# apache/bifromq

Measured on AMD Instinct MI355X. Metric: publish-topic matches/sec (whole node), higher is better.
Workload: dtype u32

## Files before the change

### bifromq_amd/csrc/bmq_dist_kernels.h

```cpp
#pragma once
#ifndef BMQ_WAVE_EMU
#include <hip/hip_runtime.h>
#endif

#include <type_traits>

#include "bmq_layout.h"
#include "bmq_batch_args.h"

namespace bmq {

#ifndef BMQ_WAVE_EMU
__device__ __forceinline__ void wave_sync() {
    __builtin_amdgcn_fence(__ATOMIC_RELEASE, "wavefront");
    __builtin_amdgcn_wave_barrier();
    __builtin_amdgcn_fence(__ATOMIC_ACQUIRE, "wavefront");
}
__device__ __forceinline__ uint32_t rank_below(unsigned long long mask) {
    return __builtin_amdgcn_mbcnt_hi((uint32_t)(mask >> 32), __builtin_amdgcn_mbcnt_lo((uint32_t)mask, 0u));
}
#endif
__device__ __forceinline__ uint32_t wave_excl_scan(uint32_t v, uint32_t lane, uint32_t& total) {
    uint32_t inc = v;
#pragma unroll
// ... 2 lines not shown
        if (lane >= (uint32_t)d) inc += o;
    }
    total = __shfl(inc, 63);
    return inc - v;
}
__device__ __forceinline__ unsigned long long wave_sum_u64(unsigned long long v) {
#pragma unroll
    for (int d = 32; d >= 1; d >>= 1) v += __shfl_xor(v, d);
    return v;
}

__device__ __forceinline__ TrieSlot unpack_slot(const uint4& a, const uint4& b) {
    TrieSlot s;
    s.parent = a.x; s.token = a.y; s.own_begin = a.z; s.own_count = a.w;
    s.hash_begin = b.x; s.hash_count = b.y; s.node = b.z; s.lit_bloom = b.w;
    return s;
}
struct Line64 {
    uint4 a0, a1, b0, b1;
};
static_assert(DICT_GROUP == 2, "a dictionary group is one Line64");
#ifndef BMQ_WAVE_EMU
__device__ __forceinline__ void load_line64(const void* p, Line64& r) {
    asm volatile("global_load_dwordx4 %0, %4, off\n\t"
                 "global_load_dwordx4 %1, %4, off offset:16\n\t"
                 "global_load_dwordx4 %2, %4, off offset:32\n\t"
                 "global_load_dwordx4 %3, %4, off offset:48\n\t"
                 "s_waitcnt vmcnt(0)"
                 : "=&v"(r.a0), "=&v"(r.a1), "=&v"(r.b0), "=&v"(r.b1)
                 : "v"(p));
}
__device__ __forceinline__ void load_line64_s(const void* sbase, uint32_t voff, Line64& r) {
    asm volatile("global_load_dwordx4 %0, %4, %5\n\t"
                 "global_load_dwordx4 %1, %4, %5 offset:16\n\t"
                 "global_load_dwordx4 %2, %4, %5 offset:32\n\t"
                 "global_load_dwordx4 %3, %4, %5 offset:48\n\t"
                 "s_waitcnt vmcnt(0)"
                 : "=&v"(r.a0), "=&v"(r.a1), "=&v"(r.b0), "=&v"(r.b1)
                 : "v"(voff), "s"(sbase));
}
#else
inline void load_line64(const void* p, Line64& r) { memcpy(&r, p, 64); }
inline void load_line64_s(const void* sbase, uint32_t voff, Line64& r) { memcpy(&r, reinterpret_cast<const uint8_t*>(sbase) + voff, 64); }
#endif
template <class ByteAt>
__device__ __forceinline__ uint32_t dict_lookup(const DistIndexView& ix, const LevelHash& h, uint32_t len,
                                                const uint32_t inl[4], uint32_t start, ByteAt&& byte_at) {
    const uint32_t tag = level_hash_tag(h);
    uint32_t g = level_hash_slot(h, len) & ix.dict_group_mask;
    auto tail_eq = [&](uint32_t pool_off) {
        bool eq = true;
        for (uint32_t i = 16; i < len && eq; i++) eq = ix.pool[pool_off + i] == byte_at(start + i);
        return eq;
    };
    for (uint32_t probes = 0; probes <= ix.dict_group_mask; probes++) {
        Line64 ln;
        load_line64(ix.dict + DICT_GROUP * (size_t)g, ln);
        const bool h0 = ln.a0.x == tag && ln.a0.z == len && ln.a1.x == inl[0] && ln.a1.y == inl[1] && ln.a1.z == inl[2] &&
                        ln.a1.w == inl[3];
        const bool h1 = ln.b0.x == tag && ln.b0.z == len && ln.b1.x == inl[0] && ln.b1.y == inl[1] && ln.b1.z == inl[2] &&
                        ln.b1.w == inl[3];
        if (h0 && (len <= 16 || tail_eq(ln.a0.w))) return ln.a0.y;
        if (h1 && (len <= 16 || tail_eq(ln.b0.w))) return ln.b0.y;
        if (ln.a0.x == 0 || ln.b0.x == 0) return TOK_UNKNOWN;
        g = (g + 1) & ix.dict_group_mask;
    }
    return TOK_UNKNOWN;
}

#ifndef BMQ_WAVE_EMU
__device__ __forceinline__ void load_slot32(const void* p, uint4& a, uint4& b) {
    asm volatile("global_load_dwordx4 %0, %2, off\n\t"
                 "global_load_dwordx4 %1, %2, off offset:16\n\t"
                 "s_waitcnt vmcnt(0)"
                 : "=&v"(a), "=&v"(b)
                 : "v"(p));
}
#else
inline void load_slot32(const void* p, uint4& a, uint4& b) {
    memcpy(&a, p, 16);
    memcpy(&b, reinterpret_cast<const uint8_t*>(p) + 16, 16);
}
#endif
template <class ByteAt>
__device__ __forceinline__ uint32_t dict_lookup_by_slot(const DistIndexView& ix, const LevelHash& h, uint32_t len, const uint32_t inl[4], uint32_t start,
                                                        ByteAt&& byte_at) {
    const uint32_t tag = level_hash_tag(h);
    uint32_t g = level_hash_slot(h, len) & ix.dict_group_mask;
    auto tail_eq = [&](uint32_t pool_off) {
        bool eq = true;
        for (uint32_t i = 16; i < len && eq; i++) eq = ix.pool[pool_off + i] == byte_at(start + i);
        return eq;
    };
    for (uint32_t probes = 0; probes <= ix.dict_group_mask; probes++) {
        const DictSlot* grp = ix.dict + DICT_GROUP * (size_t)g;
#pragma unroll
        for (uint32_t k = 0; k < DICT_GROUP; k++) {
            uint4 hd, in;
            load_slot32(grp + k, hd, in);
            if (hd.x == tag && hd.z == len && in.x == inl[0] && in.y == inl[1] && in.z == inl[2] && in.w == inl[3] && (len <= 16 || tail_eq(hd.w))) return hd.y;
            if (hd.x == 0) return TOK_UNKNOWN;
        }
        g = (g + 1) & ix.dict_group_mask;
    }
    return TOK_UNKNOWN;
}

template <class WordAt>
__device__ __forceinline__ void scan_level(uint32_t& pos, uint32_t end, bool split, WordAt&& word_at, LevelHash& h,
                                           uint32_t inl[4], uint32_t& len, bool& last) {
    h = level_hash_init();
    inl[0] = inl[1] = inl[2] = inl[3] = 0;
    len = 0;
    for (;;) {
        const uint32_t remaining = end - pos;
        if (remaining == 0) break;
        const uint32_t w = word_at(pos);
        uint32_t nb = 4;
        if (split) {
            const uint32_t x = w ^ 0x2F2F2F2Fu;
            const uint32_t z = (x - 0x01010101u) & ~x & 0x80808080u;
            if (z) nb = (uint32_t)(__ffs((int)z) - 1) >> 3;
        }
        nb = min(nb, remaining);
        if (nb) {
            const uint32_t wm = nb == 4 ? w : (w & ((1u << (8u * nb)) - 1u));
            level_hash_word(h, wm);
            if (len < 16) inl[len >> 2] = wm;
            len += nb;
            pos += nb;
        }
        if (nb < 4) break;
    }
    if (pos < end) {
        pos++;
        last = false;
    } else {
        last = true;
    }
}

__device__ __forceinline__ uint32_t global_word_at(const uint8_t* base, uint32_t p) {
    const uint32_t* a = reinterpret_cast<const uint32_t*>(base + (p & ~3u));
    return __builtin_amdgcn_alignbyte(a[1], a[0], p & 3u);
}

constexpr TenantSlot EMPTY_TENANT{0, 0, 0, 0, 0, 1, 0, 0, 0, 0, 0, 0, {0, 0, 0}, NONE};
__device__ __forceinline__ bool tenant_known(const TenantSlot& t) { return (t.hash_lo | t.hash_hi) != 0; }

__global__ __launch_bounds__(64) void k_reset(Counters* ctr, SubAlloc* subs, unsigned long long* super_sums, uint32_t n_super) {
    const uint32_t i = blockIdx.x * 64 + threadIdx.x;
    if (i < sizeof(Counters) / 8) reinterpret_cast<unsigned long long*>(ctr)[i] = 0ull;
    if (i < sizeof(SubAlloc) * 2 * N_SUB / 8) reinterpret_cast<unsigned long long*>(subs)[i] = 0ull;
    if (i < n_super) super_sums[(size_t)i * SUPER_STRIDE] = 0ull;
}

static_assert(sizeof(Counters) % 16 == 0 && sizeof(Counters) / 16 <= 64, "one wave copies the counters, 16 bytes per lane");
__global__ __launch_bounds__(64) void k_publish(const Counters* ctr, Counters* host) {
    const uint32_t i = threadIdx.x;
    if (i < sizeof(Counters) / 16) reinterpret_cast<uint4*>(host)[i] = reinterpret_cast<const uint4*>(ctr)[i];
}

struct TenantQuery {
    uint32_t beg = 0, len = 0;
    uint32_t raw[5] = {0, 0, 0, 0, 0};
    uint32_t w[4] = {0, 0, 0, 0};
// ... 367 lines not shown
```

### bifromq_amd/csrc/bmq_engine.hip

```cpp
#include <hip/hip_runtime.h>

#include <algorithm>
#include <array>
#include <chrono>
#include <condition_variable>
#include <cstdio>
#include <cstdlib>
#include <cstring>
#include <map>
#include <memory>
#include <mutex>
#include <string>
#include <string_view>
#include <thread>
#include <type_traits>
#include <vector>

#include "../../include/bmq.h"
#include "bmq_codec.h"
#include "bmq_dist_index.h"
#include "bmq_dist_kernels.h"
#include "bmq_poll_kernel.h"
#include "bmq_exec_dev.h"
#include "bmq_exec_host.h"
// ... 508 lines not shown
    S.pair_cap = S.pair_cap * 2;
    if (S.pair_cap >= 0xFFFFFFFFull) return set_err(e, BMQ_E_RANGE, "matched-range buffer exceeds 2^32 entries");
    HIPCHK(e, S.b_pairs.ensure(sizeof(MatchRange) * S.pair_cap));
    return BMQ_OK;
}
int grow_sort_list(bmq_engine* e, bmq_engine::BatchSlot& S, uint32_t sort_count) {
    S.sort_cap = std::max<uint32_t>(S.sort_cap * 2, sort_count);
    HIPCHK(e, S.b_sort_list.ensure(sizeof(uint32_t) * S.sort_cap));
    return BMQ_OK;
}

static void print_wave_debug(bmq_engine* e, bmq_engine::BatchSlot& S) {
    const BatchArgs& a = S.last;
    if (!a.dbg_wave || !a.n_blocks) return;
    std::vector<uint4> h(2 * (size_t)a.n_blocks);
    if (hipMemcpy(h.data(), a.dbg_wave, sizeof(uint4) * 2 * a.n_blocks, hipMemcpyDeviceToHost) != hipSuccess) return;
    if (a.debug_flags & 24u) {
        std::vector<std::pair<unsigned long long, int>> ev;
        unsigned long long t0 = ~0ull, t1 = 0, busy = 0;
        std::map<uint32_t, std::vector<std::pair<unsigned long long, int>>> per_simd;
        for (uint32_t i = 0; i < a.n_blocks; i++) {
            const unsigned long long st = ((unsigned long long)h[i].y << 32) | h[i].x, en = st + h[i].z;
            t0 = std::min(t0, st), t1 = std::max(t1, en), busy += h[i].z;
            ev.push_back({st, 1}), ev.push_back({en, -1});
            const uint32_t simd_key = (h[i].w >> 4) & 0xFFFFFu & ~0xCu;
            per_simd[simd_key].push_back({st, 1}), per_simd[simd_key].push_back({en, -1});
        }
        if (const char* fn = bmq_env("BMQ_CENSUS_FILE")) {
            if (FILE* f = fopen(fn, "wb")) {
                fwrite(h.data(), sizeof(uint4), a.n_blocks, f);
                fclose(f);
            }
        }
        std::sort(ev.begin(), ev.end());
        int cur = 0, peak = 0;
        for (auto& x : ev) cur += x.second, peak = std::max(peak, cur);
        int simd_peak = 0;
        double simd_peak_sum = 0;
        for (auto& kv : per_simd) {
            std::sort(kv.second.begin(), kv.second.end());
            int c = 0, pk = 0;
            for (auto& x : kv.second) c += x.second, pk = std::max(pk, c);
            simd_peak = std::max(simd_peak, pk), simd_peak_sum += pk;
        }
        fprintf(stderr, "[bmq] k_walk census: %u waves, span %llu ticks, mean wave %.0f ticks, mean resident %.0f (peak %d) waves; %zu distinct SIMD keys, peak waves on one SIMD %d (mean of peaks %.1f)\n",
                a.n_blocks, t1 - t0, (double)busy / a.n_blocks, (double)busy / (double)(t1 - t0), peak, per_simd.size(), simd_peak,
                simd_peak_sum / std::max<size_t>(per_simd.size(), 1));
        return;
    }
    if (a.debug_flags & 4u) {
        if (!BMQ_EXP_CLOCKS) {
            fprintf(stderr, "[bmq] k_expand phase clocks need a build with -DBMQ_EXP_CLOCKS=1 (tools/build_variant.sh)\n");
            return;
        }
        double p[4] = {0, 0, 0, 0};
        for (uint32_t i = 0; i < a.n_blocks; i++) p[0] += h[i].x, p[1] += h[i].y, p[2] += h[i].z, p[3] += h[i].w;
        fprintf(stderr, "[bmq] k_expand waves=%u clocks/wave: head %.0f load+order %.0f prefix %.0f generate %.0f\n", a.n_blocks,
                p[0] / a.n_blocks, p[1] / a.n_blocks, p[2] / a.n_blocks, p[3] / a.n_blocks);
        {
            std::vector<unsigned long long> tot(a.n_blocks);
            unsigned long long mx_tail = 0;
            for (uint32_t i = 0; i < a.n_blocks; i++) {
                tot[i] = (unsigned long long)h[i].x + h[i].y + h[i].z + h[i].w;
                if (i >= a.n_blocks - a.n_blocks / 10) mx_tail = std::max(mx_tail, tot[i]);
            }
            std::sort(tot.begin(), tot.end());
            fprintf(stderr, "[bmq] k_expand wave lifetimes (clocks): p50 %llu p90 %llu p99 %llu max %llu; longest among the last tenth of the blocks %llu\n",
                    tot[a.n_blocks / 2], tot[(size_t)(a.n_blocks * 0.9)], tot[(size_t)(a.n_blocks * 0.99)], tot.back(), mx_tail);
        }
        return;
    }
    double s1 = 0, s2 = 0, s3 = 0, sr = 0, si = 0;
    std::vector<uint32_t> r(a.n_blocks), c2(a.n_blocks);
    for (uint32_t i = 0; i < a.n_blocks; i++) {
        s1 += h[i].x, s2 += h[i].y, s3 += h[i].z, sr += h[i].w & 255u, si += h[i].w >> 8;
        r[i] = h[i].w & 255u, c2[i] = h[i].y;
    }
    std::sort(r.begin(), r.end());
    std::sort(c2.begin(), c2.end());
    const double n = a.n_blocks;
    {
        double pa = 0, pb = 0, pc = 0;
        for (uint32_t i = 0; i < a.n_blocks; i++) pa += h[a.n_blocks + i].x, pb += h[a.n_blocks + i].y, pc += h[a.n_blocks + i].z;
        fprintf(stderr, "[bmq] k_walk tokenise in detail: stage bytes %.0f | offsets + tenant %.0f | levels + dictionary %.0f\n", pa / n, pb / n, pc / n);
    }
    fprintf(stderr, "[bmq] k_walk waves=%u clocks/wave: tokenise %.0f walk %.0f (p50 %u p99 %u) write %.0f | rounds mean %.1f p50 %u p99 %u max %u | items/wave %.0f\n",
            a.n_blocks, s1 / n, s2 / n, c2[a.n_blocks / 2], c2[(size_t)(a.n_blocks * 0.99)], s3 / n, sr / n, r[a.n_blocks / 2],
            r[(size_t)(a.n_blocks * 0.99)], r.back(), si / n);
}

int finish_dist(bmq_engine* e, bmq_engine::BatchSlot& S, uint64_t* out_total) {
    const auto rerun = [&] {
        BatchArgs a = S.last;
        return launch_dist(e, S, a);
    };
    for (int attempt = 0; attempt < 8; attempt++) {
        HIPCHK(e, hipEventSynchronize(S.ev_done));
        if (S.last.debug_flags & 30u) print_wave_debug(e, S);
        const Counters c = *S.h_ctr;
        const uint32_t grow = c.status & (ST_RERUN | ST_NEED_SORTLIST | ST_NEED_ADJ);
        if (grow) {
            int rc;
            if ((grow & ST_NEED_PAIRS) && (rc = grow_pairs(e, S))) return rc;
            if (grow & ST_NEED_SPILL) {
                S.spill_cap = S.spill_cap * 2;
                if (S.spill_cap >= 0xFFFFFFFFull) return set_err(e, BMQ_E_RANGE, "range spill buffer exceeds 2^32 records");
                HIPCHK(e, S.b_spill.ensure(sizeof(uint4) * S.spill_cap));
            }
            if (grow & ST_NEED_SLOW) {
                S.slow_cap = std::max<uint32_t>(S.slow_cap * 2, c.slow_count);
                HIPCHK(e, S.b_slow_list.ensure(sizeof(uint32_t) * S.slow_cap));
            }
            if (grow & ST_NEED_SCRATCH) {
                S.scratch_cap = std::max<uint64_t>(S.scratch_cap * 2, c.scratch_alloc + c.scratch_alloc / 8);
                HIPCHK(e, S.b_scratch.ensure(sizeof(uint32_t) * S.scratch_cap));
            }
            if (grow & ST_NEED_ADJ) {
                S.adj_cap = (uint64_t)c.adj_bytes + c.adj_bytes / 8 + 4096;
                HIPCHK(e, S.b_c_topics.ensure(S.adj_cap + 64));
            }
            if ((grow & ST_NEED_SORTLIST) && (rc = grow_sort_list(e, S, c.sort_count))) return rc;
            if (c.sort_count) e->sort_on = true, e->sort_idle = 0;
            if (c.slow_count) e->slow_on = true, e->slow_idle = 0;
            if (c.status & ST_WANT_MIXED) e->mixed_on = true, e->mixed_idle = 0;
            if ((rc = rerun())) return rc;
            continue;
        }
        if ((c.status & ST_WANT_MIXED) && !S.ran_mixed) {
            e->mixed_on = true, e->mixed_idle = 0;
            if (int rc = rerun()) return rc;
            continue;
        }
        if (c.slow_count && !S.ran_slow) {
            e->slow_on = true, e->slow_idle = 0;
            if (int rc = rerun()) return rc;
            continue;
        }
        if (c.sort_count && !S.ran_sort && !(c.status & (ST_RANGE | ST_NOSPACE))) {
            e->sort_on = true, e->sort_idle = 0;
            HIPCHK(e, hipMemcpyAsync(S.last.ctr, S.h_ctr, sizeof(Counters), hipMemcpyHostToDevice, e->stream));
            hipLaunchKernelGGL(k_sort_rows, dim3(1024), dim3(256), 0, e->stream, S.last);
            reset_slot(e, S, e->stream);
            HIPCHK(e, hipGetLastError());
            HIPCHK(e, hipStreamSynchronize(e->stream));
        }
        if (S.ran_slow && (c.slow_count ? (e->slow_idle = 0) : ++e->slow_idle) >= REPAIR_IDLE_BATCHES) e->slow_on = false;
        if (S.ran_sort && (c.sort_count ? (e->sort_idle = 0) : ++e->sort_idle) >= REPAIR_IDLE_BATCHES) e->sort_on = false;
        if (S.ran_mixed && ++e->mixed_idle >= 8 * REPAIR_IDLE_BATCHES) e->mixed_on = false;
        S.pending = false;
        bmq_stats& st = e->stats;
        st = bmq_stats{};
        st.n_topics = S.last.n_topics;
        st.n_visit = c.n_visit;
        st.n_match = c.total_ids;
        st.n_ranges = c.n_ranges;
        st.n_slow_topics = c.slow_count;
        st.n_sorted_rows = c.sort_count;
        st.topic_bytes = c.topic_bytes;
        st.n_walked = c.n_walked ? c.n_walked : (S.last.rep ? 0u : S.last.n_topics);
        st.n_split_blocks = S.last.heavy_list ? std::min(c.heavy_count, S.last.heavy_cap) : 0u;
        if (S.last.heavy_list) {
            const double nb = S.last.n_blocks, mr = c.n_ranges / nb, mi = c.total_ids / nb;
            e->blk_mean_ranges = e->blk_mean_ranges > 0 ? 0.75 * e->blk_mean_ranges + 0.25 * mr : mr;
            e->blk_mean_ids = e->blk_mean_ids > 0 ? 0.75 * e->blk_mean_ids + 0.25 * mi : mi;
            constexpr double base = EXPAND_SPLIT_MULT_X16 / 16.0;
            if (c.heavy_count > S.last.heavy_cap) e->split_mult *= 1.25;
            else if (c.heavy_count < S.last.heavy_cap / 4) e->split_mult = std::max(base, e->split_mult / 1.05);
// ... 1359 lines not shown
```

### bifromq_amd/csrc/bmq_walk_kernel.h

```cpp
#pragma once

namespace bmq {

constexpr uint32_t WALK_MAX_TENANTS = 4;
__device__ __forceinline__ uint32_t walk_meta(uint32_t tl, uint32_t tokpos, uint32_t rem) { return tl | (tokpos << 6) | (rem << 16); }
constexpr uint32_t WALK_META_CHILD = 64u - 65536u;

#define BMQ_WALK_GEOM_DEFAULT 512, 176, 152
#define BMQ_WALK_GEOM_SMALLEST 192, 128, 128
constexpr uint32_t WALK_QC_DEFAULT = 176, WALK_PC_DEFAULT = 152, WALK_QC_SMALLEST = 128, WALK_PC_SMALLEST = 128;

template <int TC, int QC, int PC, bool MIXED> struct WalkLds {
    static constexpr uint32_t TOK = 0;
    static constexpr uint32_t STK = TOK + TC * 4;
    static constexpr uint32_t PRG = STK + QC * 8;
    static constexpr uint32_t PTP = PRG + PC * 8;
    static constexpr uint32_t VIS = PTP + PC;
    static constexpr uint32_t REG = VIS + 64 * 4;
    static constexpr uint32_t BYTES = (REG + (MIXED ? 64 * 8 : 0) + 15) & ~15u;
    static constexpr uint32_t STAGE = BYTES - STK;
    static constexpr uint32_t ALLOC = (BYTES + 511) & ~511u;
#ifndef BMQ_WALK_MAX_WAVES
#define BMQ_WALK_MAX_WAVES 8
#endif
    static constexpr uint32_t WAVES_LDS = (163840 / ALLOC) / 4 > BMQ_WALK_MAX_WAVES ? BMQ_WALK_MAX_WAVES : (163840 / ALLOC) / 4;
    static constexpr uint32_t WAVES = MIXED && WAVES_LDS > 5 ? 5 : WAVES_LDS;
    static_assert(3 * 64 * 4 <= STK && PC % 8 == 0 && QC % 8 == 0 && STK % 16 == 0 && WAVES >= 1 && TC >= 2 * FAST_LEVELS && TC <= 1023, "layout");
    static_assert(FAST_LEVELS <= 32, "walk_meta keeps the levels behind an item in 5 bits");
    static_assert(QC >= 128 && PC >= 128, "one sink pushes up to 128 items and emits up to 128 ranges into an empty list");
    static_assert(STK + (QC + 64) * 8 <= BYTES, "a round reads 64 stack slots from `tail` on, whatever is there");
};

#ifdef BMQ_WAVE_EMU
struct WalkCoverage {
    unsigned long long flushes = 0, parks = 0, restores = 0;
    unsigned long long tails = 0, tail_levels = 0, tail_leaves = 0;
    unsigned long long tail_reach[TAIL_K + 1][2] = {}, tail_stop[TAIL_K + 1][2][TAIL_K] = {}, tail_short[TAIL_K + 1][2][TAIL_K] = {};
    unsigned long long tail_plus[TAIL_K] = {}, tombs = 0;
    unsigned long long cf_spared[3] = {}, cf_ones[3] = {};
};
inline WalkCoverage walk_cov;
#define BMQ_WALK_COV(field) do { if (threadIdx.x == 0) walk_cov.field++; } while (0)
#else
#define BMQ_WALK_COV(field) do { } while (0)
#endif

#ifndef BMQ_WAVE_EMU
__device__ __forceinline__ uint32_t lane_here() {
    uint32_t v = threadIdx.x;
    asm volatile("" : "+v"(v));
    return v;
}
__device__ __forceinline__ uint32_t sgpr(uint32_t v) { return __builtin_amdgcn_readfirstlane(v); }
__device__ __forceinline__ unsigned long long ballot64(bool p) { return __builtin_amdgcn_ballot_w64(p); }
#endif

template <int TC, int QC, int PC, bool MIXED>
__device__ __forceinline__ void walk_wave(const BatchArgs& a, const uint32_t block_x, uint32_t* const lds) {
    using G = WalkLds<TC, QC, PC, MIXED>;
    uint32_t* const tokens = lds + G::TOK / 4;
    uint2* const stk = reinterpret_cast<uint2*>(lds + G::STK / 4);
    uint2* const p_rng = reinterpret_cast<uint2*>(lds + G::PRG / 4);
    uint8_t* const p_topic = reinterpret_cast<uint8_t*>(lds) + G::PTP;
    uint32_t* const cnt_visit = lds + G::VIS / 4;
    uint2* const t_region = reinterpret_cast<uint2*>(lds + G::REG / 4);
    uint32_t* const cnt_pairs = lds + G::TOK / 4;
    uint32_t* const cnt_routes = cnt_pairs + 64;
    uint32_t* const cursor = cnt_routes + 64;

    const uint32_t lane = threadIdx.x;
    uint32_t blk;
    if (BMQ_DBG(a, 32u)) {
        const uint32_t per = (a.n_blocks + 7u) >> 3;
        blk = (block_x & 7u) * per + (per - 1u - (block_x >> 3));
        if ((block_x >> 3) >= per || blk >= a.n_blocks) return;
    } else {
        if (block_x >= a.n_blocks) return;
        blk = BMQ_DBG(a, 256u) ? block_x : a.n_blocks - 1 - block_x;
    }
    const uint32_t tpw = 1u << a.tpw_shift;
    const uint32_t t = (blk << a.tpw_shift) + lane;
    const bool valid = lane < tpw && t < a.n_topics;
    const bool dbg_w = BMQ_DBG(a, 2u) && a.dbg_wave;
    const unsigned long long clk0 = dbg_w ? __builtin_amdgcn_s_memtime() : 0ull;
    const unsigned long long clk0c = (BMQ_DBG(a, 8u) && a.dbg_wave) ? __builtin_amdgcn_s_memtime() : 0ull;

    const uint32_t t_first = blk << a.tpw_shift, t_end = min(t_first + tpw, a.n_topics);
    const uint32_t s_beg = scalar_words(a.topic_off)[t_first], s_end = scalar_words(a.topic_off)[t_end];
    const uint32_t a0 = s_beg & ~15u;
    const bool staged = (s_end - a0) + 32u <= G::STAGE;
    if (staged) {
        uint4* dst = reinterpret_cast<uint4*>(stk);
        const uint4* src = reinterpret_cast<const uint4*>(a.topics + a0);
        const uint32_t n16 = (s_end - a0 + 15) >> 4;
        for (uint32_t o = lane; o < n16; o += 64) dst[o] = src[o];
    }
    uint32_t nlev = 0, pos = 0, end = 0, ti = 0xFFFFFFFFu;
    if (valid) {
        pos = a.topic_off[t];
        end = a.topic_off[t + 1];
        ti = a.topic_tenant[t];
    }
    const bool asked = ti < a.n_tenants && (a.rep == nullptr || a.rep[t] == t);
    wave_sync();
    const uint8_t* lbytes = reinterpret_cast<const uint8_t*>(stk);
    const uint32_t* lwords = reinterpret_cast<const uint32_t*>(stk);
    const uint8_t* gbytes = a.topics;
    if (asked) {
        uint32_t cnt = 1;
        for (uint32_t p = pos & ~3u; p < end; p += 4) {
            const uint32_t w = staged ? lwords[(p - a0) >> 2] : *reinterpret_cast<const uint32_t*>(gbytes + p);
            const uint32_t x = w ^ 0x2F2F2F2Fu;
            uint32_t z = ~(((x & 0x7F7F7F7Fu) + 0x7F7F7F7Fu) | x | 0x7F7F7F7Fu);
            if (p < pos) z &= 0xFFFFFFFFu << (8u * (pos - p));
            if (p + 4 > end) z &= 0xFFFFFFFFu >> (8u * (p + 4 - end));
            cnt += (uint32_t)__popc(z);
        }
        nlev = cnt;
    }
    const bool deep = nlev > (uint32_t)FAST_LEVELS;
    const bool sys = asked && end > pos && (staged ? (uint32_t)lbytes[pos - a0] : (uint32_t)gbytes[pos]) == '$';
    const unsigned long long clkA = dbg_clock(dbg_w);
    uint32_t tok_base = 0;
    auto tokenise = [&](bool mine, bool from_lds) {
        auto byte_at = [&](uint32_t i) -> uint32_t { return from_lds ? (uint32_t)lbytes[i - a0] : (uint32_t)gbytes[i]; };
        auto word_at = [&](uint32_t i) -> uint32_t {
            if (!from_lds) return global_word_at(gbytes, i);
            const uint32_t rel = i - a0;
            return __builtin_amdgcn_alignbyte(lwords[(rel >> 2) + 1], lwords[rel >> 2], rel & 3u);
        };
        bool more = mine;
        uint32_t p = pos;
        for (uint32_t l = 0; ballot64(more) != 0; l++) {
            LevelHash h = level_hash_init();
            uint32_t inl[4] = {0, 0, 0, 0}, len = 0;
            const uint32_t start = p;
            const bool now = more;
            if (more) {
                bool last;
                scan_level(p, end, true, word_at, h, inl, len, last);
                more = !last;
            }
            const uint32_t tok = now ? (BMQ_DBG(a, 128u) ? dict_lookup(a.ix, h, len, inl, start, byte_at) : dict_lookup_by_slot(a.ix, h, len, inl, start, byte_at))
                                     : TOK_UNKNOWN;
            if (now) tokens[tok_base + l] = tok;
        }
    };

    uint32_t tail = 0, pcount = 0, rounds = 0, items = 0;
    const uint32_t f_off = a.ix.filter_off;
    uint32_t fl_base = 0, fl_len = 0;
    uint32_t qs_base = 0, qs_len = 0;
    auto spill_alloc = [&](const BatchArgs& c, uint32_t ln, uint32_t n, uint32_t& base) -> bool {
        unsigned long long sb = 0;
        uint32_t ok = 1;
        if (ln == 0) ok = pair_alloc(c.subs + N_SUB, c.spill_cap, blk, n + 1, sb) ? 1u : 0u;
        const uint32_t lo = sgpr((uint32_t)sb), hi = sgpr((uint32_t)(sb >> 32));
        const bool fits = sgpr(ok) != 0 && hi == 0 && lo + n + 1 < 0xFFFFFFFFu && lo + n + 1 > lo;
        if (!fits && ln == 0) atomicOr(&c.ctr->status, ST_NEED_SPILL);
        base = lo;
        return fits;
    };
    const unsigned long long clk1 = dbg_clock(dbg_w);
    auto sink = [&](uint32_t own_begin, uint32_t own_count , uint32_t hash_begin, uint32_t hash_count ,
                    uint32_t lit , uint32_t bloom , uint32_t child,
                    uint32_t cmeta , uint32_t tl, uint32_t ln ) {
        const bool emit_own = own_count != 0, emit_hash = hash_count != 0, push_l = lit != 0, push_h = (int32_t)bloom < 0;
        const unsigned long long m_own = ballot64(emit_own), m_hash = ballot64(emit_hash);
        const unsigned long long m_l = ballot64(push_l), m_h = ballot64(push_h);
        if ((m_own | m_hash) != 0) {
            const uint32_t n_own = (uint32_t)__popcll(m_own), n_emit = n_own + (uint32_t)__popcll(m_hash);
            if (__builtin_expect(pcount + n_emit > (uint32_t)PC, 0)) {
                const BatchArgs& c = a;
                BMQ_WALK_COV(flushes);
                uint32_t cb;
                if (spill_alloc(c, ln, pcount, cb)) {
                    if (ln == 0) c.spill[cb] = make_uint4(fl_base, fl_len, 0u, 0u);
                    for (uint32_t i = ln; i < pcount; i += 64) c.spill[cb + 1 + i] = make_uint4(p_rng[i].x, p_rng[i].y, p_topic[i], 0u);
                    fl_base = cb;
                    fl_len = pcount;
                }
                pcount = 0;
                wave_sync();
            }
            if (emit_own) {
                const uint32_t p = pcount + rank_below(m_own);
                p_rng[p] = make_uint2(own_begin, own_count);
                p_topic[p] = (uint8_t)tl;
            }
            if (emit_hash) {
                const uint32_t p = pcount + n_own + rank_below(m_hash);
                p_rng[p] = make_uint2(hash_begin, hash_count);
                p_topic[p] = (uint8_t)tl;
            }
            pcount += n_emit;
        }
        if ((m_l | m_h) != 0) {
            const uint32_t n_l = (uint32_t)__popcll(m_l), n_push = n_l + (uint32_t)__popcll(m_h);
            if (__builtin_expect(tail + n_push > (uint32_t)QC, 0)) {
                const BatchArgs& c = a;
                BMQ_WALK_COV(parks);
                uint32_t cb;
                if (spill_alloc(c, ln, tail, cb)) {
                    if (ln == 0) c.spill[cb] = make_uint4(qs_base, qs_len, 0u, 0u);
                    for (uint32_t i = ln; i < tail; i += 64) c.spill[cb + 1 + i] = make_uint4(stk[i].x, stk[i].y, 0u, 0u);
                    qs_base = cb;
                    qs_len = tail;
                }
                tail = 0;
                wave_sync();
            }
            if (push_l) stk[tail + rank_below(m_l)] = make_uint2(child, cmeta);
            if (push_h) stk[tail + n_l + rank_below(m_h)] = make_uint2(child, cmeta | KIND_P);
            tail += n_push;
        }
        wave_sync();
    };
    auto drain = [&](auto mode_tag, const TrieSlot* s_rptr, uint32_t s_rbuckets) {
        constexpr int MODE = decltype(mode_tag)::value;
        while ((tail | qs_len) != 0) {
            const uint32_t ln = lane_here();
            if (__builtin_expect(tail == 0, 0)) {
                const BatchArgs& c = a;
                BMQ_WALK_COV(restores);
                const uint32_t hx = sgpr(c.spill[qs_base].x), hy = sgpr(c.spill[qs_base].y);
                for (uint32_t i = ln; i < qs_len; i += 64) {
                    const uint4 r = c.spill[qs_base + 1 + i];
                    stk[i] = make_uint2(r.x, r.y);
// ... 74 lines not shown
                q_own_count = (reach && !is_hash && rem == k) ? cnt : 0u;
                p_hash_begin = p_own_begin, p_hash_count = (reach && is_hash) ? cnt : 0u, p_bloom = 0u;
#ifdef BMQ_WAVE_EMU
                {
                    const uint32_t kind = is_hash ? 1u : 0u, rr[TAIL_K] = {r0, r1, r2, r3};
                    if (reach && (q_own_count | p_hash_count) != 0) walk_cov.tail_reach[k][kind]++;
                    else if (n_tail < k) (rem == n_tail ? walk_cov.tail_short : walk_cov.tail_stop)[k][kind][n_tail]++;
                    for (uint32_t j = 0; j < n_tail && j < TAIL_K; j++) walk_cov.tail_plus[j] += rr[j] == TOK_PLUS;
                }
#endif
            } else {
                const uint32_t ph = tnext2 * FILTER_MUL;
                const uint32_t pf = (((p_own_count | f_off) != 0 ? FILTER_NONE : p_own_begin) >> (ph >> 27)) & (((p_hash_count | f_off) != 0 ? FILTER_NONE : p_hash_begin) >> ((ph >> 22) & 31u));
#ifdef BMQ_WAVE_EMU
                if (plus_here && !p_last && f_off == 0) {
                    walk_cov.cf_spared[2] += tnext2 != 0 && ((p_bloom >> bloom_bit(tnext2)) & 1u) != 0 && (pf & 1u) == 0;
                    walk_cov.cf_ones[2] += (p_own_count == 0 && p_own_begin == FILTER_NONE) || (p_hash_count == 0 && p_hash_begin == FILTER_NONE);
                }
#endif
                p_hash_count = plus_here ? p_hash_count : 0u;
                p_bloom = (plus_here && !p_last) ? ((p_bloom & BLOOM_PLUS) | min((p_bloom >> bloom_bit(tnext2)) & pf & 1u, tnext2)) : 0u;
            }
            if (found) atomicAdd(&cnt_visit[tl], (plus_here ? 2u : 1u) + n_tail);
#ifdef BMQ_WAVE_EMU
            if (tail_here) walk_cov.tails++, walk_cov.tail_levels += n_tail, walk_cov.tail_leaves += (q_own_count | p_hash_count) != 0;
#endif
            uint32_t e_own_begin = own_begin, e_own_count = (found && last) ? own_count : 0u, e_hash_begin = hash_begin;
            uint32_t e_hash_count = found ? hash_count : 0u;
            const uint32_t fh = tnext * FILTER_MUL;
            const uint32_t f_lit = (((own_count | f_off) != 0 ? FILTER_NONE : own_begin) >> (fh >> 27)) & (((hash_count | f_off) != 0 ? FILTER_NONE : hash_begin) >> ((fh >> 22) & 31u));
            uint32_t e_lit = tail_here ? 0u : min((bloom_in >> bloom_bit(tnext)) & f_lit & 1u, tnext), e_bloom = (plus_here || tail_here) ? 0u : bloom_in;
            uint32_t e_child = child, e_meta = cmeta;
#ifdef BMQ_WAVE_EMU
            if (found && !last && !tail_here && f_off == 0) {
                walk_cov.cf_spared[1] += tnext != 0 && ((bloom_in >> bloom_bit(tnext)) & 1u) != 0 && (f_lit & 1u) == 0;
                walk_cov.cf_ones[1] += (own_count == 0 && own_begin == FILTER_NONE) || (hash_count == 0 && hash_begin == FILTER_NONE);
            }
#endif
            const bool second = ballot64(plus_here || tail_here) != 0;
#pragma clang loop unroll(disable)
            for (uint32_t part = 0;; part++) {
                sink(e_own_begin, e_own_count, e_hash_begin, e_hash_count, e_lit, e_bloom, e_child, e_meta, tl, ln);
                if (part == 1 || !second) break;
                e_own_begin = p_own_begin, e_own_count = q_own_count, e_hash_begin = p_hash_begin, e_hash_count = p_hash_count;
                e_lit = p_bloom & 1u, e_bloom = p_bloom, e_child = p_node, e_meta = cmeta + WALK_META_CHILD;
            }
        }
    };
    struct RootPlus {
        uint32_t has;
        uint4 p0;
        uint2 p0n;
        uint4 pp0;
        uint2 pp0n;
    };
    auto boot = [&](bool mine, uint32_t r_hash_begin, uint32_t r_hash_count, uint32_t r_bloom, const RootPlus& rp) {
        const uint32_t ln = lane_here();
        bool actp = mine;
#pragma clang loop unroll(disable)
        for (uint32_t part = 0; part <= rp.has; part++) {
            const uint4 pl = part == 0 ? make_uint4(0u, 0u, r_hash_begin, r_hash_count) : (part == 1 ? rp.p0 : rp.pp0);
            const uint32_t nd = part == 0 ? 0u : (part == 1 ? rp.p0n.x : rp.pp0n.x), bl = part == 0 ? r_bloom : (part == 1 ? rp.p0n.y : rp.pp0n.y);
            const uint32_t tk = tokens[actp ? tok_base + part : 0u];
            const bool root_sys = part == 0 && sys;
            const uint32_t bloom_in = (actp && nlev > part) ? bl : 0u;
            const uint32_t f_own = (part == 0 || (pl.y | f_off) != 0) ? FILTER_NONE : pl.x, f_hash = (part == 0 || (pl.w | f_off) != 0) ? FILTER_NONE : pl.z;
            const uint32_t fh = tk * FILTER_MUL;
            if (part != 0 && actp) cnt_visit[ln] += 1u;
#ifdef BMQ_WAVE_EMU
            if (part != 0 && actp && nlev > part && f_off == 0) {
                const uint32_t s_own = fh >> 27, s_hash = (fh >> 22) & 31u;
                walk_cov.cf_spared[0] += tk != 0 && ((bloom_in >> bloom_bit(tk)) & 1u) != 0 && (((f_own >> s_own) & (f_hash >> s_hash)) & 1u) == 0;
                walk_cov.cf_ones[0] += (pl.y == 0 && pl.x == FILTER_NONE) || (pl.w == 0 && pl.z == FILTER_NONE);
            }
#endif
            sink(pl.x, (actp && nlev == part) ? pl.y : 0u ,
                 pl.z, (actp && !root_sys) ? pl.w : 0u, min((bloom_in >> bloom_bit(tk)) & (f_own >> (fh >> 27)) & (f_hash >> ((fh >> 22) & 31u)) & 1u, tk),
                 (root_sys || part < rp.has) ? (bloom_in & ~BLOOM_PLUS) : bloom_in,
                 nd, walk_meta(ln, tok_base + part, nlev - 1 - part), ln, ln);
            actp = actp && !root_sys && (int32_t)bloom_in < 0;
            if (ballot64(actp) == 0) break;
        }
    };
    {
    const BatchArgs& b = a;
    const bool run = !BMQ_DBG(b, 1u);
    uint2 t_region_early = make_uint2(0u, 1u);
    uint32_t m_hash_begin = 0, m_hash_count = 0, m_bloom = 0;
    if (MIXED) {
        uint2 reg = make_uint2(0u, 1u);
        if (asked) {
            const TenantSlot rg = resolve_tenant(b, ti);
            if (tenant_known(rg)) reg = make_uint2(rg.base, rg.buckets), m_hash_begin = rg.root_hash_begin, m_hash_count = rg.root_hash_count, m_bloom = rg.root_lit_bloom;
        }
        t_region_early = reg;
    }
    unsigned long long left = ballot64(asked && !deep);
    if (left == 0) cnt_visit[lane] = 0;
    for (bool first = true; left != 0; first = false) {
        const bool cand = (left >> lane) & 1ull;
        uint32_t total;
        tok_base = wave_excl_scan(cand ? nlev : 0u, lane, total);
        const unsigned long long chunk = ballot64(cand && tok_base + nlev <= (uint32_t)TC);
        left &= ~chunk;
        const bool mine = (chunk >> lane) & 1ull;
        tokenise(mine, first && staged);
        if (first) cnt_visit[lane] = 0;
        wave_sync();
        if (!run) continue;
        if (MIXED) {
            if (first) {
                t_region[lane] = t_region_early;
                wave_sync();
            }
            boot(mine, m_hash_begin, m_hash_count, m_bloom, RootPlus{0u, make_uint4(0u, 0u, 0u, 0u), make_uint2(0u, 0u), make_uint4(0u, 0u, 0u, 0u), make_uint2(0u, 0u)});
            drain(std::integral_constant<int, 2>{}, b.ix.trie, 1u);
        } else {
            unsigned long long todo = chunk;
            for (uint32_t n_seg = 0; todo != 0; n_seg++) {
                if (n_seg == WALK_MAX_TENANTS) {
                    if (lane == 0) atomicOr(&b.ctr->status, ST_WANT_MIXED);
                    left = 0;
                    break;
                }
                const uint32_t cur = (uint32_t)__builtin_amdgcn_readlane((int)ti, (int)__builtin_ctzll(todo));
                const unsigned long long seg = ballot64(mine && ti == cur);
                todo &= ~seg;
                const TenantSlot rg = resolve_tenant_uniform(b, cur);
                if (!tenant_known(rg)) continue;
                const uint32_t s_rbase = sgpr(rg.base), s_rbuckets = sgpr(rg.buckets);
                RootPlus rp{0u, make_uint4(0u, 0u, 0u, 0u), make_uint2(0u, 0u), make_uint4(0u, 0u, 0u, 0u), make_uint2(0u, 0u)};
                const uint32_t s_rplus = sgpr(rg.root_plus);
                if ((int32_t)sgpr(rg.root_lit_bloom) < 0 && s_rplus != NONE) {
                    ScalarWords sp = scalar_words(b.ix.trie + (size_t)s_rbase + (s_rplus & ~1u));
                    const uint32_t o0 = (s_rplus & 1u) * 8u, o1 = 8u - o0;
                    rp.has = 1u, rp.p0 = make_uint4(sp[o0 + 2], sp[o0 + 3], sp[o0 + 4], sp[o0 + 5]), rp.p0n = make_uint2(sp[o0 + 6], sp[o0 + 7]);
                    if (sp[o1] == rp.p0n.x && sp[o1 + 1] == TOK_PLUS)
                        rp.has = 2u, rp.pp0 = make_uint4(sp[o1 + 2], sp[o1 + 3], sp[o1 + 4], sp[o1 + 5]), rp.pp0n = make_uint2(sp[o1 + 6], sp[o1 + 7]);
                }
                boot(mine && ti == cur, sgpr(rg.root_hash_begin), sgpr(rg.root_hash_count), sgpr(rg.root_lit_bloom), rp);
                if (s_rbuckets < (1u << 25)) drain(std::integral_constant<int, 0>{}, b.ix.trie + s_rbase, s_rbuckets);
                else drain(std::integral_constant<int, 1>{}, b.ix.trie + s_rbase, s_rbuckets);
            }
        }
    }
    }

    const unsigned long long clk2 = dbg_clock(dbg_w);
    const BatchArgs& d = a;
    const uint32_t l3 = lane_here();
    const uint32_t t3_first = blk << d.tpw_shift, t3 = t3_first + l3;
    const bool valid3 = l3 < (1u << d.tpw_shift) && t3 < d.n_topics;
    cnt_pairs[l3] = 0;
    cnt_routes[l3] = 0;
    wave_sync();
    for (uint32_t cb = fl_base, cl = fl_len; cl != 0;) {
        const uint32_t hx = sgpr(d.spill[cb].x), hy = sgpr(d.spill[cb].y);
        for (uint32_t i = l3; i < cl; i += 64) {
            const uint4 r = d.spill[cb + 1 + i];
            atomicAdd(&cnt_pairs[r.z], 1u);
            atomicAdd(&cnt_routes[r.z], r.y & ~RANGE_INDIRECT);
        }
        cb = hx;
        cl = hy;
    }
    for (uint32_t i = l3; i < pcount; i += 64) {
        const uint32_t tp = p_topic[i];
        atomicAdd(&cnt_pairs[tp], 1u);
        atomicAdd(&cnt_routes[tp], p_rng[i].y & ~RANGE_INDIRECT);
    }
    wave_sync();
    const bool flagged = deep;
    const uint32_t np = flagged ? 0u : cnt_pairs[l3];
    const uint32_t nr = flagged ? 0u : cnt_routes[l3];
    uint32_t total_pairs;
    const uint32_t excl = wave_excl_scan(np, l3, total_pairs);
    total_pairs = sgpr(total_pairs);
    unsigned long long base = 0;
    uint32_t fits_l = 1;
    if (l3 == 0 && total_pairs) fits_l = pair_alloc(d.subs, d.pair_cap, blk, total_pairs, base) ? 1u : 0u;
    base = ((unsigned long long)sgpr((uint32_t)(base >> 32)) << 32) | sgpr((uint32_t)base);
    const bool fits = sgpr(fits_l) != 0;
    if (!fits && l3 == 0) atomicOr(&d.ctr->status, ST_NEED_PAIRS);
    cursor[l3] = excl;
    wave_sync();
    if (fits && total_pairs) {
        auto copy_chunk = [&](uint32_t cb, uint32_t cl) {
            for (uint32_t i = l3; i < cl; i += 64) {
                const uint4 r = d.spill[cb + 1 + i];
                const uint32_t dst = atomicAdd(&cursor[r.z], 1u);
                d.pairs[base + dst] = MatchRange{r.x, r.y};
            }
        };
        uint32_t n_ch = 0;
        for (uint32_t cb = fl_base, cl = fl_len; cl != 0;) {
            const uint32_t hx = sgpr(d.spill[cb].x), hy = sgpr(d.spill[cb].y);
            if (n_ch < (uint32_t)QC) {
                stk[n_ch] = make_uint2(cb, cl);
                n_ch++;
            } else copy_chunk(cb, cl);
            cb = hx;
            cl = hy;
        }
        wave_sync();
        while (n_ch != 0) {
            n_ch--;
            copy_chunk(sgpr(stk[n_ch].x), sgpr(stk[n_ch].y));
        }
        for (uint32_t i = l3; i < pcount; i += 64) {
            const uint32_t dst = atomicAdd(&cursor[p_topic[i]], 1u);
            const uint2 r = p_rng[i];
            d.pairs[base + dst] = MatchRange{r.x, r.y};
        }
    }
    if (valid3) {
        d.pair_off[t3] = (uint32_t)(base + excl);
        d.pair_cnt[t3] = np;
        d.route_cnt[t3] = nr;
        if (flagged && ti < d.n_tenants) {
            const uint32_t sp = atomicAdd(&d.ctr->slow_count, 1u);
            if (sp < d.slow_cap) d.slow_list[sp] = t3;
            else atomicOr(&d.ctr->status, ST_NEED_SLOW);
        }
    }
    const uint32_t vis = cnt_visit[l3];
    if (valid3 && d.visit_cnt) d.visit_cnt[t3] = vis;
    const unsigned long long wsum = wave_sum_u64(nr);
    const unsigned long long wvis = wave_sum_u64(vis);
    const unsigned long long wbytes = scalar_words(d.topic_off)[min(t3_first + (1u << d.tpw_shift), d.n_topics)] - scalar_words(d.topic_off)[t3_first];
    if (l3 == 0) {
        if (d.rep == nullptr) {
            d.wave_sums[blk] = wsum;
            if (wsum) atomicAdd(&d.super_sums[(size_t)(blk >> SUPER_SHIFT) * SUPER_STRIDE], wsum);
            d.blk_stats[blk] = make_uint4((uint32_t)wvis, total_pairs, (uint32_t)wbytes, heavy_mark(d, blk, total_pairs, wsum));
        }
        if (BMQ_DBG(d, 8u) && d.dbg_wave) {
            const unsigned long long clk3 = __builtin_amdgcn_s_memtime();
            const uint32_t hw = __builtin_amdgcn_s_getreg((4 << 0) | (0 << 6) | (31 << 11));
            const uint32_t xcc = __builtin_amdgcn_s_getreg((20 << 0) | (0 << 6) | (31 << 11));
            d.dbg_wave[blk] = make_uint4((uint32_t)clk0c, (uint32_t)(clk0c >> 32), (uint32_t)(clk3 - clk0c), (hw & 0xFFFFu) | (xcc << 16));
        }
        if (dbg_w) {
            const unsigned long long clk3 = __builtin_amdgcn_s_memtime();
            d.dbg_wave[blk] = make_uint4((uint32_t)(clk1 - clk0), (uint32_t)(clk2 - clk1), (uint32_t)(clk3 - clk2), rounds | (items << 8));
            d.dbg_wave[d.n_blocks + blk] = make_uint4((uint32_t)(clkA - clk0), 0u, (uint32_t)(clk1 - clkA), 0u);
        }
    }
}

template <int TC, int QC, int PC, bool MIXED>
__global__ __launch_bounds__(64, (WalkLds<TC, QC, PC, MIXED>::WAVES)) void k_walk(BatchArgs a) {
    __shared__ __align__(16) uint32_t lds[WalkLds<TC, QC, PC, MIXED>::BYTES / 4];
    walk_wave<TC, QC, PC, MIXED>(a, blockIdx.x, lds);
}

#if BMQ_EXPERIMENTS
__global__ __launch_bounds__(64, 8) void k_occ_probe(BatchArgs a) {
    __shared__ uint32_t lds[5024 / 4];
    asm volatile("s_mov_b32 s71, 0" ::: "s71");
    asm volatile("v_mov_b32 v63, 0" ::: "v63");
    const unsigned long long t0 = __builtin_amdgcn_s_memtime();
    lds[threadIdx.x] = a.n_topics;
    while (__builtin_amdgcn_s_memtime() - t0 < 100000u) __builtin_amdgcn_s_sleep(8);
    const uint32_t acc = lds[(threadIdx.x + 1) & 63];
    const unsigned long long t1 = __builtin_amdgcn_s_memtime();
    if (threadIdx.x == 0 && blockIdx.x < a.n_blocks) {
        const uint32_t hw = __builtin_amdgcn_s_getreg((4 << 0) | (0 << 6) | (31 << 11));
        const uint32_t xcc = __builtin_amdgcn_s_getreg((20 << 0) | (0 << 6) | (31 << 11));
        a.dbg_wave[blockIdx.x] = make_uint4((uint32_t)t0, (uint32_t)(t0 >> 32), (uint32_t)(t1 - t0) | (acc == 0x1234567u), (hw & 0xFFFFu) | (xcc << 16));
    }
}

#endif

}
```

Baseline: 3.975 billion.

## Tokenise topic levels across lanes with pipelined dictionary probes

Replaces per-lane level counting and tokenising with a wave-cooperative pass. It scans the staged topic bytes in 16-byte pieces, builds a bitmap of level boundaries, and uses a prefix scan to write every level's start and end straight into LDS. Each lane then hashes one level and issues its first dictionary slot load without waiting. Several such requests stay in flight before they are resolved, so global-memory latency is overlapped instead of serialised per lane. The new path runs only on the first chunk when topics are staged, no topic is deep and the levels fit in TC; otherwise it falls back to the old code. It adds LDS atomics, extra scans and more code complexity.

After: 4.017 billion, median of 3. No clear change (+1.1%).

```diff
diff --git a/bifromq_amd/csrc/bmq_dist_kernels.h b/bifromq_amd/csrc/bmq_dist_kernels.h
--- a/bifromq_amd/csrc/bmq_dist_kernels.h
+++ b/bifromq_amd/csrc/bmq_dist_kernels.h
@@ -108,6 +108,33 @@
     memcpy(&b, reinterpret_cast<const uint8_t*>(p) + 16, 16);
 }
 #endif
+#ifndef BMQ_WAVE_EMU
+__device__ __forceinline__ void load_slot32_nowait(const void* p, uint4& a, uint4& b) {
+    a = reinterpret_cast<const uint4*>(p)[0];
+    b = reinterpret_cast<const uint4*>(p)[1];
+}
+#else
+inline void load_slot32_nowait(const void* p, uint4& a, uint4& b) { load_slot32(p, a, b); }
+#endif
+template <class ByteAt>
+__device__ __forceinline__ uint32_t dict_lookup_from_slot0(const DistIndexView& ix, uint32_t tag, uint32_t g, uint32_t len, const uint32_t inl[4], uint32_t start,
+                                                           uint4 hd, uint4 in, ByteAt&& byte_at) {
+    auto tail_eq = [&](uint32_t pool_off) {
+        bool eq = true;
+        for (uint32_t i = 16; i < len && eq; i++) eq = ix.pool[pool_off + i] == byte_at(start + i);
+        return eq;
+    };
+    for (uint32_t probes = 0, k = 0;;) {
+        if (hd.x == tag && hd.z == len && in.x == inl[0] && in.y == inl[1] && in.z == inl[2] && in.w == inl[3] && (len <= 16 || tail_eq(hd.w))) return hd.y;
+        if (hd.x == 0) return TOK_UNKNOWN;
+        if (++k == DICT_GROUP) {
+            k = 0;
+            g = (g + 1) & ix.dict_group_mask;
+            if (++probes > ix.dict_group_mask) return TOK_UNKNOWN;
+        }
+        load_slot32(ix.dict + DICT_GROUP * (size_t)g + k, hd, in);
+    }
+}
 template <class ByteAt>
 __device__ __forceinline__ uint32_t dict_lookup_by_slot(const DistIndexView& ix, const LevelHash& h, uint32_t len, const uint32_t inl[4], uint32_t start,
                                                         ByteAt&& byte_at) {
diff --git a/bifromq_amd/csrc/bmq_engine.hip b/bifromq_amd/csrc/bmq_engine.hip
--- a/bifromq_amd/csrc/bmq_engine.hip
+++ b/bifromq_amd/csrc/bmq_engine.hip
@@ -614,7 +614,8 @@
     {
         double pa = 0, pb = 0, pc = 0;
         for (uint32_t i = 0; i < a.n_blocks; i++) pa += h[a.n_blocks + i].x, pb += h[a.n_blocks + i].y, pc += h[a.n_blocks + i].z;
-        fprintf(stderr, "[bmq] k_walk tokenise in detail: stage bytes %.0f | offsets + tenant %.0f | levels + dictionary %.0f\n", pa / n, pb / n, pc / n);
+        fprintf(stderr, "[bmq] k_walk tokenise in detail: stage bytes + offsets + level list %.0f | set-up %.0f | hash + dictionary %.0f (%.1f %% of the wave's clocks; all of tokenise %.1f %%)\n",
+                pa / n, pb / n, pc / n, 100.0 * pc / (s1 + s2 + s3), 100.0 * s1 / (s1 + s2 + s3));
     }
     fprintf(stderr, "[bmq] k_walk waves=%u clocks/wave: tokenise %.0f walk %.0f (p50 %u p99 %u) write %.0f | rounds mean %.1f p50 %u p99 %u max %u | items/wave %.0f\n",
             a.n_blocks, s1 / n, s2 / n, c2[a.n_blocks / 2], c2[(size_t)(a.n_blocks * 0.99)], s3 / n, sr / n, r[a.n_blocks / 2],
diff --git a/bifromq_amd/csrc/bmq_walk_kernel.h b/bifromq_amd/csrc/bmq_walk_kernel.h
--- a/bifromq_amd/csrc/bmq_walk_kernel.h
+++ b/bifromq_amd/csrc/bmq_walk_kernel.h
@@ -31,6 +31,10 @@
     static_assert(STK + (QC + 64) * 8 <= BYTES, "a round reads 64 stack slots from `tail` on, whatever is there");
 };
 
+#ifndef BMQ_TOK_FLIGHT
+#define BMQ_TOK_FLIGHT 2
+#endif
+enum { TOKF_UNSTAGED, TOKF_NO_ROOM, TOKF_UNASKED, TOKF_EMPTY, TOKF_DEEP, TOKF_CHUNKED, TOKF_REASONS };
 #ifdef BMQ_WAVE_EMU
 struct WalkCoverage {
     unsigned long long flushes = 0, parks = 0, restores = 0;
@@ -38,8 +42,10 @@
     unsigned long long tail_reach[TAIL_K + 1][2] = {}, tail_stop[TAIL_K + 1][2][TAIL_K] = {}, tail_short[TAIL_K + 1][2][TAIL_K] = {};
     unsigned long long tail_plus[TAIL_K] = {}, tombs = 0;
     unsigned long long cf_spared[3] = {}, cf_ones[3] = {};
+    unsigned long long tok_lanes = 0, tok_unaligned = 0, tok_fallback[TOKF_REASONS] = {}, tok_later_chunks = 0, tok_checked = 0, tok_mismatch = 0;
 };
 inline WalkCoverage walk_cov;
+inline bool walk_tok_check = false;
 #define BMQ_WALK_COV(field) do { if (threadIdx.x == 0) walk_cov.field++; } while (0)
 #else
 #define BMQ_WALK_COV(field) do { } while (0)
@@ -54,6 +60,8 @@
 __device__ __forceinline__ uint32_t sgpr(uint32_t v) { return __builtin_amdgcn_readfirstlane(v); }
 __device__ __forceinline__ unsigned long long ballot64(bool p) { return __builtin_amdgcn_ballot_w64(p); }
 #endif
+
+__device__ __forceinline__ uint32_t wave_incl_scan(uint32_t v);
 
 template <int TC, int QC, int PC, bool MIXED>
 __device__ __forceinline__ void walk_wave(const BatchArgs& a, const uint32_t block_x, uint32_t* const lds) {
@@ -106,18 +114,90 @@
     const uint8_t* lbytes = reinterpret_cast<const uint8_t*>(stk);
     const uint32_t* lwords = reinterpret_cast<const uint32_t*>(stk);
     const uint8_t* gbytes = a.topics;
-    if (asked) {
+    auto slash_bytes = [](uint32_t w) -> uint32_t {
+        const uint32_t x = w ^ 0x2F2F2F2Fu;
+        return ~(((x & 0x7F7F7F7Fu) + 0x7F7F7F7Fu) | x | 0x7F7F7F7Fu);
+    };
+    auto count_levels = [&]() -> uint32_t {
+        if (!asked) return 0u;
         uint32_t cnt = 1;
         for (uint32_t p = pos & ~3u; p < end; p += 4) {
-            const uint32_t w = staged ? lwords[(p - a0) >> 2] : *reinterpret_cast<const uint32_t*>(gbytes + p);
-            const uint32_t x = w ^ 0x2F2F2F2Fu;
-            uint32_t z = ~(((x & 0x7F7F7F7Fu) + 0x7F7F7F7Fu) | x | 0x7F7F7F7Fu);
+            uint32_t z = slash_bytes(staged ? lwords[(p - a0) >> 2] : *reinterpret_cast<const uint32_t*>(gbytes + p));
             if (p < pos) z &= 0xFFFFFFFFu << (8u * (pos - p));
             if (p + 4 > end) z &= 0xFFFFFFFFu >> (8u * (p + 4 - end));
             cnt += (uint32_t)__popc(z);
         }
-        nlev = cnt;
-    }
+        return cnt;
+    };
+    uint16_t* const tok16 = reinterpret_cast<uint16_t*>(tokens);
+    bool lanes_ok = false;
+    uint32_t n_events = 0;
+    {
+        const uint32_t rb = s_beg - a0, re = s_end - a0;
+        const uint32_t n_piece = (re >> 4) + 1;
+        const uint32_t map_off = (n_piece + 1) << 4;
+        const uint32_t map_words = (n_piece + 1) >> 1;
+        const bool room = staged && map_off + map_words * 4 <= G::STAGE;
+        const unsigned long long m_unasked = ballot64(valid && !asked), m_empty = ballot64(valid && asked && end == pos);
+        if (!staged) BMQ_WALK_COV(tok_fallback[TOKF_UNSTAGED]);
+        else if (!room) BMQ_WALK_COV(tok_fallback[TOKF_NO_ROOM]);
+        else if (m_unasked != 0) BMQ_WALK_COV(tok_fallback[TOKF_UNASKED]);
+        else if (m_empty != 0) BMQ_WALK_COV(tok_fallback[TOKF_EMPTY]);
+        if (room && (m_unasked | m_empty) == 0 && !BMQ_DBG(a, 128u)) {
+            uint32_t* const endmap = lds + (G::STK + map_off) / 4;
+            const uint16_t* const endmap16 = reinterpret_cast<const uint16_t*>(endmap);
+            for (uint32_t o = lane; o < map_words; o += 64) endmap[o] = 0;
+            wave_sync();
+            const uint32_t e_rel = end - a0, e_piece = e_rel >> 4, e_below = (1u << (e_rel & 15u)) - 1u;
+            if (valid) atomicOr(&endmap[e_rel >> 5], 1u << (e_rel & 31u));
+            if (lane == 0) tok16[0] = (uint16_t)rb;
+            wave_sync();
+            uint32_t carry = 0, rank_end = 0;
+            for (uint32_t o0 = 0; o0 < n_piece; o0 += 64) {
+                const uint32_t o = o0 + lane;
+                uint32_t sb = 0, eb = 0;
+                if (o < n_piece) {
+                    const uint4 q = reinterpret_cast<const uint4*>(stk)[o];
+                    auto nibble = [&](uint32_t w) -> uint32_t {
+                        const uint32_t z = slash_bytes(w) >> 7;
+                        return (z | (z >> 7) | (z >> 14) | (z >> 21)) & 15u;
+                    };
+                    sb = nibble(q.x) | (nibble(q.y) << 4) | (nibble(q.z) << 8) | (nibble(q.w) << 12);
+                    const uint32_t lo = max(rb, o << 4) - (o << 4), hi = min(re, (o << 4) + 16u) - (o << 4);
+                    sb = (int32_t)hi > (int32_t)lo ? sb & ((1u << hi) - 1u) & ~((1u << lo) - 1u) : 0u;
+                    eb = endmap16[o];
+                }
+                const uint32_t n_here = (uint32_t)__popc(sb) + (uint32_t)__popc(eb), n_incl = wave_incl_scan(n_here);
+                const uint32_t base = carry + n_incl - n_here;
+                const uint32_t there = __shfl((base << 16) | sb, e_piece & 63u);
+                if (valid && (e_piece >> 6) == (o0 >> 6))
+                    rank_end = (there >> 16) + (uint32_t)__popc(there & 0xFFFFu & e_below) + (uint32_t)__popc((uint32_t)endmap16[e_piece] & e_below);
+                for (uint32_t rem = sb; ballot64(rem != 0) != 0;) {
+                    if (rem != 0) {
+                        const uint32_t b = (uint32_t)__ffs((int)rem) - 1u;
+                        rem &= rem - 1u;
+                        const uint32_t j = base + (uint32_t)__popc(sb & ((1u << b) - 1u)) + (uint32_t)__popc(eb & ((2u << b) - 1u)), p_rel = (o << 4) + b;
+                        if (j < (uint32_t)TC) tok16[2 * j + 1] = (uint16_t)p_rel;
+                        if (j + 1 < (uint32_t)TC) tok16[2 * j + 2] = (uint16_t)(p_rel + 1);
+                    }
+                }
+                carry += (uint32_t)__builtin_amdgcn_readlane((int)n_incl, 63);
+            }
+            if (valid) {
+                if (rank_end < (uint32_t)TC) tok16[2 * rank_end + 1] = (uint16_t)e_rel;
+                if (rank_end + 1 < (uint32_t)TC) tok16[2 * rank_end + 2] = (uint16_t)e_rel;
+            }
+            const uint32_t rank_prev = __shfl_up(rank_end, 1);
+            nlev = valid ? (lane == 0 ? rank_end + 1 : rank_end - rank_prev) : 0u;
+            n_events = carry;
+            lanes_ok = true;
+            wave_sync();
+#ifdef BMQ_WAVE_EMU
+            if (walk_tok_check && nlev != count_levels()) walk_cov.tok_mismatch++;
+#endif
+        }
+    }
+    if (!lanes_ok) nlev = count_levels();
     const bool deep = nlev > (uint32_t)FAST_LEVELS;
     const bool sys = asked && end > pos && (staged ? (uint32_t)lbytes[pos - a0] : (uint32_t)gbytes[pos]) == '$';
     const unsigned long long clkA = dbg_clock(dbg_w);
@@ -144,6 +224,49 @@
             const uint32_t tok = now ? (BMQ_DBG(a, 128u) ? dict_lookup(a.ix, h, len, inl, start, byte_at) : dict_lookup_by_slot(a.ix, h, len, inl, start, byte_at))
                                      : TOK_UNKNOWN;
             if (now) tokens[tok_base + l] = tok;
+        }
+    };
+    auto tokenise_lanes = [&]() {
+        struct Group {
+            uint32_t desc, tag, g, i0, i1, i2, i3;
+            uint4 hd, in;
+        };
+        auto byte_at = [&](uint32_t rel) -> uint32_t { return (uint32_t)lbytes[rel]; };
+        auto request = [&](Group& s, uint32_t j) {
+            s.desc = j < n_events ? tokens[j] : 0u;
+            const uint32_t start = s.desc & 0xFFFFu, len = (s.desc >> 16) - start;
+            LevelHash h = level_hash_init();
+            s.i0 = s.i1 = s.i2 = s.i3 = 0;
+            for (uint32_t off = 0; ballot64(off < len) != 0; off += 4) {
+                if (off < len) {
+                    const uint32_t rel = start + off, left = len - off;
+                    const uint32_t w = __builtin_amdgcn_alignbyte(lwords[(rel >> 2) + 1], lwords[rel >> 2], rel & 3u);
+                    const uint32_t wm = left >= 4 ? w : (w & ((1u << (8u * left)) - 1u));
+                    level_hash_word(h, wm);
+                    if (off == 0) s.i0 = wm;
+                    else if (off == 4) s.i1 = wm;
+                    else if (off == 8) s.i2 = wm;
+                    else if (off == 12) s.i3 = wm;
+                }
+            }
+            s.tag = level_hash_tag(h);
+            s.g = level_hash_slot(h, len) & a.ix.dict_group_mask;
+            load_slot32_nowait(a.ix.dict + DICT_GROUP * (size_t)s.g, s.hd, s.in);
+        };
+        auto resolve = [&](Group& s, uint32_t j) {
+            const uint32_t start = s.desc & 0xFFFFu, len = (s.desc >> 16) - start;
+            const uint32_t inl[4] = {s.i0, s.i1, s.i2, s.i3};
+            if (j < n_events) tokens[j] = dict_lookup_from_slot0(a.ix, s.tag, s.g, len, inl, start, s.hd, s.in, byte_at);
+        };
+        Group s[BMQ_TOK_FLIGHT];
+#pragma unroll
+        for (uint32_t d = 0; d + 1 < BMQ_TOK_FLIGHT; d++) request(s[d], 64 * d + lane);
+        for (uint32_t j0 = 0; j0 < n_events; j0 += 64 * BMQ_TOK_FLIGHT) {
+#pragma unroll
+            for (uint32_t d = 0; d < BMQ_TOK_FLIGHT; d++) {
+                request(s[(d + BMQ_TOK_FLIGHT - 1) % BMQ_TOK_FLIGHT], j0 + 64 * (d + BMQ_TOK_FLIGHT - 1) + lane);
+                resolve(s[d], j0 + 64 * d + lane);
+            }
         }
     };
 
@@ -384,6 +507,7 @@
             if (ballot64(actp) == 0) break;
         }
     };
+    unsigned long long clk_tok = 0;
     {
     const BatchArgs& b = a;
     const bool run = !BMQ_DBG(b, 1u);
@@ -398,6 +522,10 @@
         t_region_early = reg;
     }
     unsigned long long left = ballot64(asked && !deep);
+    const unsigned long long any_deep = ballot64(deep);
+#ifdef BMQ_WAVE_EMU
+    const unsigned long long left_all = left;
+#endif
     if (left == 0) cnt_visit[lane] = 0;
     for (bool first = true; left != 0; first = false) {
         const bool cand = (left >> lane) & 1ull;
@@ -406,7 +534,35 @@
         const unsigned long long chunk = ballot64(cand && tok_base + nlev <= (uint32_t)TC);
         left &= ~chunk;
         const bool mine = (chunk >> lane) & 1ull;
-        tokenise(mine, first && staged);
+        const unsigned long long clk_t = dbg_clock(dbg_w);
+        if (first && lanes_ok && any_deep == 0 && n_events <= (uint32_t)TC) {
+            BMQ_WALK_COV(tok_lanes);
+            if (s_beg != a0) BMQ_WALK_COV(tok_unaligned);
+            tokenise_lanes();
+#ifdef BMQ_WAVE_EMU
+            if (walk_tok_check) {
+                static uint32_t seen[TC];
+                static uint32_t seen_base[64];
+                wave_sync();
+                for (uint32_t j = lane; j < n_events; j += 64) seen[j] = tokens[j], tokens[j] = 0xDEADBEEFu;
+                uint32_t rank_total;
+                seen_base[lane] = wave_excl_scan(count_levels(), lane, rank_total);
+                wave_sync();
+                tokenise(mine, true);
+                wave_sync();
+                bool same = seen_base[lane] == tok_base && chunk == left_all && rank_total == n_events;
+                for (uint32_t j = lane; j < n_events; j += 64) same = same && seen[j] == tokens[j];
+                if (ballot64(!same) != 0) BMQ_WALK_COV(tok_mismatch);
+                BMQ_WALK_COV(tok_checked);
+            }
+#endif
+        } else {
+            if (!first) BMQ_WALK_COV(tok_later_chunks);
+            else if (lanes_ok && any_deep != 0) BMQ_WALK_COV(tok_fallback[TOKF_DEEP]);
+            else if (lanes_ok) BMQ_WALK_COV(tok_fallback[TOKF_CHUNKED]);
+            tokenise(mine, first && staged);
+        }
+        clk_tok += dbg_clock(dbg_w) - clk_t;
         if (first) cnt_visit[lane] = 0;
         wave_sync();
         if (!run) continue;
@@ -544,8 +700,8 @@
         }
         if (dbg_w) {
             const unsigned long long clk3 = __builtin_amdgcn_s_memtime();
-            d.dbg_wave[blk] = make_uint4((uint32_t)(clk1 - clk0), (uint32_t)(clk2 - clk1), (uint32_t)(clk3 - clk2), rounds | (items << 8));
-            d.dbg_wave[d.n_blocks + blk] = make_uint4((uint32_t)(clkA - clk0), 0u, (uint32_t)(clk1 - clkA), 0u);
+            d.dbg_wave[blk] = make_uint4((uint32_t)(clk1 - clk0 + clk_tok), (uint32_t)(clk2 - clk1 - clk_tok), (uint32_t)(clk3 - clk2), rounds | (items << 8));
+            d.dbg_wave[d.n_blocks + blk] = make_uint4((uint32_t)(clkA - clk0), (uint32_t)(clk1 - clkA), (uint32_t)clk_tok, 0u);
         }
     }
 }
```
